# nanoporetech/tombo

Measured on NVIDIA H100. Metric: resquiggle_reads_per_sec, higher is better.
Workload: dtype f64

## Files before the change

### tombo_b200/csrc/batch.h

```cpp
#pragma once
#ifdef TB2_EMUL
#include <stddef.h>
#include "../../include/tombo_b200.h"
struct tb2_ctx;
#else
#include "ctx.h"
#endif

struct ReadState {
    int status;
    int active;
    int done;
    int n_iters;
    int calls;
    int attempt;
    int first_status;
    int use_sv;
    int num_events;
    int n_cpts;
    int rsrtr;
    int n_norm;
    int changed;
    int path;
    int mapped_start, clip;
    int n_stalls;
    int pad_;
    double shc, scc;
    double score;
    tb2_scale_values sv;
};

struct BatchView {
    int n_reads;
    int kmer_width;
    int max_raw;
    const long long *raw_off, *seq_off, *base_off, *ev_off;
    const int *order;
    const unsigned char *seq;
    double *rawf;
    double *norm;
    double *cs;
    double *scores;
    unsigned char *cstate;
    int *cpts;
    double *em;
    double *rm, *rs;
    double *bm;
    double *tmp_b;
    int *starts;
    int *read_tb;
    int *segs_dp;
    int *segs;
    int *stall_ints;
    int stall_cap;
    ReadState *st;
};

struct StagePolicy {
    double outlier_thresh;
    long long max_raw_cpts;
    double min_event_to_seq_ratio;
    double sig_match_thresh;
    int max_scaling_iters;
    int is_rna;
    int skip_seq_scaling;
    double const_scale;
    unsigned int subsample_seed;
    int literal_key;
    int read_index_base;
};

int tb2_launch_prep(tb2_ctx *ctx, const BatchView &b, const void *raw_dev, int raw_dtype,
                    int is_rna, long long total_samples, long long total_bases);
int tb2_launch_begin_call(tb2_ctx *ctx, const BatchView &b, const tb2_params &p,
                          const StagePolicy &pol);
int tb2_launch_normalize(tb2_ctx *ctx, const BatchView &b, const StagePolicy &pol, int first_call);
int tb2_launch_cpts(tb2_ctx *ctx, const BatchView &b, const tb2_params &p, int on_raw);
int tb2_launch_rna_scale(tb2_ctx *ctx, const BatchView &b, const StagePolicy &pol);
int tb2_launch_event_means(tb2_ctx *ctx, const BatchView &b);
int tb2_launch_stalls(tb2_ctx *ctx, const BatchView &b);
int tb2_launch_resolve(tb2_ctx *ctx, const BatchView &b, const tb2_params &p,
                       const StagePolicy &pol, size_t rawdp_cap_doubles);
int tb2_launch_base_means(tb2_ctx *ctx, const BatchView &b);
int tb2_launch_theil_sen(tb2_ctx *ctx, const BatchView &b, const StagePolicy &pol, int first_call);
int tb2_launch_finalize(tb2_ctx *ctx, const BatchView &b, const StagePolicy &pol, int first_call,
                        double *norm_mean_out, double *norm_signal_out);
int tb2_launch_count_active(tb2_ctx *ctx, const BatchView &b, int *dev_counter);

struct BatchResultView {
    int n_reads;
    long long total_bases;
    const double *norm_mean;
    const long long *base_off, *seq_off;
    const unsigned char *seq;
    const int *status;
    int stride;
};
int tb2_batch_result_view(tb2_ctx *ctx, BatchResultView *out);
int tb2_region_accumulate_dev(tb2_ctx *ctx, long long n, const double *stats_dev,
                              const long long *pos_dev, double thresh, double lower, int stat_type);
```

### tombo_b200/csrc/pipeline.cu

```cuda
#include "batch.h"
#include <chrono>
#include <exception>
#include <string>
#include <cstdio>
#include <cstdlib>
#include "kernels.h"
#include <algorithm>
#include <cmath>
#include <cstring>
#include <memory>
#include <vector>

int tb2_launch_start_attempt(tb2_ctx *ctx, const BatchView &b, int attempt);
int tb2_launch_end_call(tb2_ctx *ctx, const BatchView &b, int max_iters);

namespace {

enum {
    B_RAWOFF = 12, B_SEQOFF, B_BASEOFF, B_EVOFF, B_SEQ, B_RAWIN, B_RAWF, B_NORM, B_CS, B_SCORES,
    B_CSTATE, B_CPTS, B_EM, B_RM, B_RS, B_BM, B_TMPB, B_STARTS, B_READTB, B_SEGSDP, B_SEGS,
    B_STALLS, B_STATE, B_DBG, B_COUNTERS, B_OUT_SEGS, B_OUT_NORMMEAN, B_OUT_NORMSIG, B_OUT_SMALL,
    B_SVIN, B_NSTALL, B_ORDER
};

// ... 178 lines not shown
        sv[r] = s.sv;
        score[r] = ok ? s.score : NAN;
        status[r] = s.status;
        n_iters[r] = s.n_iters;
        flags[r] = (s.changed ? 1 : 0) | (s.attempt ? 2 : 0) | ((dbg && dbg[3 * r] == 0) ? 4 : 0);
    }
}

StagePolicy stage_policy(const tb2_policy &pl)
{
    StagePolicy sp;
    sp.outlier_thresh = pl.outlier_thresh;
    sp.max_raw_cpts = pl.max_raw_cpts;
    sp.min_event_to_seq_ratio = pl.min_event_to_seq_ratio;
    sp.sig_match_thresh = pl.sig_match_thresh;
    sp.max_scaling_iters = (int)pl.max_scaling_iters;
    sp.is_rna = (int)pl.is_rna;
    sp.skip_seq_scaling = (int)pl.skip_seq_scaling;
    sp.const_scale = pl.const_scale;
    sp.subsample_seed = pl.subsample_seed;
    sp.literal_key = 0;
    sp.read_index_base = 0;
    return sp;
}

AlignBatch make_align_batch(tb2_ctx *ctx, const BatchView &v, const tb2_params &p, double thresh)
{
    AlignBatch ab;
    ab.n_reads = v.n_reads;
    ab.order = v.order;
    ab.cpts = v.cpts; ab.em = v.em; ab.ev_off = v.ev_off;
    ab.rm = v.rm; ab.rs = v.rs; ab.base_off = v.base_off;
    ab.starts = v.starts; ab.read_tb = v.read_tb; ab.segs = v.segs_dp;
    ab.stride = (int)(sizeof(ReadState) / sizeof(int));
    ab.n_cpts = &v.st[0].n_cpts;
    ab.num_events = &v.st[0].num_events;
    ab.rsrtr = &v.st[0].rsrtr;
    ab.status = &v.st[0].status;
    ab.active = &v.st[0].active;
    ab.dbg = ctx->pool[B_DBG].as<int>();
    ab.params = p;
    ab.sig_match_thresh = thresh;
    return ab;
}

int run_call(tb2_ctx *ctx, const BatchView &v, const tb2_params &p, const StagePolicy &sp,
             const AlignLaunchCfg *acfg ,
             int first_call, double *norm_mean_dev,
             double *norm_sig_dev, size_t rawdp_cap)
{
    int rc;
    if ((rc = tb2_launch_begin_call(ctx, v, p, sp))) return rc;
    if (p.use_t_test_seg) {
        if ((rc = tb2_launch_cpts(ctx, v, p, 1))) return rc;
        if ((rc = tb2_launch_rna_scale(ctx, v, sp))) return rc;
        if ((rc = tb2_launch_normalize(ctx, v, sp, first_call))) return rc;
    } else {
        if ((rc = tb2_launch_normalize(ctx, v, sp, first_call))) return rc;
        if ((rc = tb2_launch_cpts(ctx, v, p, 0))) return rc;
    }
    if ((rc = tb2_launch_event_means(ctx, v))) return rc;
    TB2_CUDA_TRY(ctx, cudaEventRecord(ctx->ev2, ctx->stream));
    for (int k = 0; k < 2; ++k)
        if (acfg[k].tb_words > 0 &&
            (rc = tb2_launch_align(ctx, make_align_batch(ctx, v, p, sp.sig_match_thresh), acfg[k])))
            return rc;
    TB2_CUDA_TRY(ctx, cudaEventRecord(ctx->ev3, ctx->stream));
    if ((rc = tb2_launch_resolve(ctx, v, p, sp, rawdp_cap))) return rc;
    if ((rc = tb2_launch_base_means(ctx, v))) return rc;
    if ((rc = tb2_launch_theil_sen(ctx, v, sp, first_call))) return rc;
    if ((rc = tb2_launch_finalize(ctx, v, sp, first_call, norm_mean_dev, norm_sig_dev))) return rc;
    if ((rc = tb2_launch_end_call(ctx, v, sp.max_scaling_iters))) return rc;
    return TB2_OK;
}

}

extern "C" int tb2_set_model(tb2_ctx *ctx, const double *means, const double *sds, int kmer_width,
                             int central_pos)
{
    int rc = tb2_use(ctx);
    if (rc) return rc;
    if (!means || !sds || kmer_width < 1 || kmer_width > 12 || central_pos < 0 ||
        central_pos >= kmer_width)
        return TB2_ERR_INVALID_ARG;
    const size_t n = (size_t)1 << (2 * kmer_width);
    TB2_CUDA_TRY(ctx, ctx->model_means.reserve(n * 8));
    TB2_CUDA_TRY(ctx, ctx->model_sds.reserve(n * 8));
    TB2_CUDA_TRY(ctx, cudaMemcpyAsync(ctx->model_means.p, means, n * 8, cudaMemcpyHostToDevice, ctx->stream));
    TB2_CUDA_TRY(ctx, cudaMemcpyAsync(ctx->model_sds.p, sds, n * 8, cudaMemcpyHostToDevice, ctx->stream));
    TB2_CUDA_TRY(ctx, cudaStreamSynchronize(ctx->stream));
    ctx->kmer_width = kmer_width;
    ctx->central_pos = central_pos;
    return TB2_OK;
}

namespace {
struct BatchHolder {
    HostBatch hb;
    BatchView v;
    std::vector<int64_t> raw_off;
    int raw_dtype = 0;
    bool uploaded = false, computed = false, has_norm_sig = false;
    bool has_sv_in = false, has_stalls_in = false;
};

BatchHolder *holder_of(tb2_ctx *ctx)
{
    if (!ctx->batch) ctx->batch = std::shared_ptr<void>(new BatchHolder(), [](void *p) { delete (BatchHolder *)p; });
    return (BatchHolder *)ctx->batch.get();
}
}

static int batch_upload_impl(tb2_ctx *ctx, int64_t n_reads, const void *raw, int raw_dtype,
// ... 426 lines not shown
    if (i < n) out[i] = in[i];
}

}

extern "C" int tb2_normalize_raw_signal(tb2_ctx *ctx, const double *raw, int64_t n, int norm_type,
                                        double outlier_thresh, double const_scale,
                                        const tb2_scale_values *sv_in, double *norm_out,
                                        tb2_scale_values *sv_out)
{
    int rc = tb2_use(ctx);
    if (rc) return rc;
    if (!raw || !norm_out || !sv_out || n < 1 || (norm_type != 0 && norm_type != 1))
        return TB2_ERR_INVALID_ARG;
    OneRead o;
    if ((rc = one_read_view(ctx, o, raw, n, 1, default_params(), 2))) return rc;
    ReadState st;
    memset(&st, 0, sizeof(st));
    st.active = 1;
    if (sv_in) { st.use_sv = 1; st.sv = *sv_in; }
    TB2_CUDA_TRY(ctx, cudaMemcpyAsync(o.v.st, &st, sizeof(st), cudaMemcpyHostToDevice, ctx->stream));
    StagePolicy sp;
    memset(&sp, 0, sizeof(sp));
    sp.outlier_thresh = outlier_thresh;
    sp.const_scale = norm_type == 1 ? const_scale : NAN;
    if ((rc = tb2_launch_normalize(ctx, o.v, sp, 1))) return rc;
    TB2_CUDA_TRY(ctx, cudaMemcpyAsync(norm_out, o.v.norm, (size_t)n * 8, cudaMemcpyDeviceToHost, ctx->stream));
    if ((rc = fetch_state(ctx, o.v, &st))) return rc;
    *sv_out = st.sv;
    if (sv_in == nullptr) sv_out->outlier_thresh = outlier_thresh;
    return st.status;
}

extern "C" int tb2_valid_cpts_w_cap(tb2_ctx *ctx, const double *sig, int64_t n,
                                    int64_t min_base_obs, int64_t running_stat_width,
                                    int64_t num_cpts, int t_test, int64_t *cpts_out,
                                    int *read_status)
{
    int rc = tb2_use(ctx);
    if (rc) return rc;
    if (!sig || !cpts_out || n < 1 || num_cpts < 1 || min_base_obs < 1 || running_stat_width < 1)
        return TB2_ERR_INVALID_ARG;
    tb2_params p = default_params();
    p.min_obs_per_base = min_base_obs;
    p.running_stat_width = running_stat_width;
    p.use_t_test_seg = t_test ? 1 : 0;
    OneRead o;
    if ((rc = one_read_view(ctx, o, sig, n, 1, p, num_cpts))) return rc;
    ReadState st;
    memset(&st, 0, sizeof(st));
    st.active = 1;
    st.num_events = (int)num_cpts;
    TB2_CUDA_TRY(ctx, cudaMemcpyAsync(o.v.st, &st, sizeof(st), cudaMemcpyHostToDevice, ctx->stream));
    if ((rc = tb2_launch_cpts(ctx, o.v, p, 1))) return rc;
    if ((rc = fetch_state(ctx, o.v, &st))) return rc;
    if (read_status) *read_status = st.status;
    if (st.status == TB2_OK) {
        std::vector<int> c32((size_t)num_cpts);
        TB2_CUDA_TRY(ctx, cudaMemcpy(c32.data(), o.v.cpts, (size_t)num_cpts * 4, cudaMemcpyDeviceToHost));
        for (int64_t i = 0; i < num_cpts; ++i) cpts_out[i] = c32[i];
    }
    return TB2_OK;
}

extern "C" int tb2_new_means(tb2_ctx *ctx, const double *sig, int64_t n_sig, const int64_t *segs,
                             int64_t n_segs, double *means_out)
{
    int rc = tb2_use(ctx);
    if (rc) return rc;
    if (!sig || !segs || !means_out || n_sig < 1 || n_segs < 1) return TB2_ERR_INVALID_ARG;
    OneRead o;
    if ((rc = one_read_view(ctx, o, nullptr, n_sig, 1, default_params(), n_segs + 1))) return rc;
    TB2_CUDA_TRY(ctx, cudaMemcpyAsync(o.v.norm, sig, (size_t)n_sig * 8, cudaMemcpyHostToDevice, ctx->stream));
    std::vector<int> s32((size_t)n_segs + 1);
    for (int64_t i = 0; i <= n_segs; ++i) {
        if (segs[i] < 0 || segs[i] > n_sig) return TB2_ERR_INVALID_ARG;
        s32[i] = (int)segs[i];
    }
    TB2_CUDA_TRY(ctx, cudaMemcpyAsync(o.v.cpts, s32.data(), (size_t)(n_segs + 1) * 4, cudaMemcpyHostToDevice, ctx->stream));
    ReadState st;
    memset(&st, 0, sizeof(st));
    st.active = 1;
    st.n_cpts = (int)n_segs + 1;
    TB2_CUDA_TRY(ctx, cudaMemcpyAsync(o.v.st, &st, sizeof(st), cudaMemcpyHostToDevice, ctx->stream));
    if ((rc = tb2_launch_event_means(ctx, o.v))) return rc;
    TB2_CUDA_TRY(ctx, cudaMemcpyAsync(means_out, o.v.em, (size_t)n_segs * 8, cudaMemcpyDeviceToHost, ctx->stream));
    TB2_CUDA_TRY(ctx, cudaStreamSynchronize(ctx->stream));
    return TB2_OK;
}

extern "C" int tb2_theil_sen(tb2_ctx *ctx, double prev_shift, double prev_scale,
                             const double *event_means, const double *model_means, int64_t n,
                             uint32_t subsample_key, double *out4, int *read_status)
{
    int rc = tb2_use(ctx);
    if (rc) return rc;
    if (!event_means || !model_means || !out4 || n < 1) return TB2_ERR_INVALID_ARG;
    OneRead o;
    if ((rc = one_read_view(ctx, o, nullptr, 1, n, default_params(), 2))) return rc;
    TB2_CUDA_TRY(ctx, cudaMemcpyAsync(o.v.bm, event_means, (size_t)n * 8, cudaMemcpyHostToDevice, ctx->stream));
    TB2_CUDA_TRY(ctx, cudaMemcpyAsync(o.v.rm, model_means, (size_t)n * 8, cudaMemcpyHostToDevice, ctx->stream));
    ReadState st;
    memset(&st, 0, sizeof(st));
    st.active = 1;
    st.sv.shift = prev_shift; st.sv.scale = prev_scale;
    TB2_CUDA_TRY(ctx, cudaMemcpyAsync(o.v.st, &st, sizeof(st), cudaMemcpyHostToDevice, ctx->stream));
    StagePolicy sp;
// ... 126 lines not shown
```

### tombo_b200/csrc/stage_kernels.cu

```cuda
#include "stage_kernels.cuh"

static inline int grid1d(int n, int bs) { return (n + bs - 1) / bs; }

int tb2_launch_prep(tb2_ctx *ctx, const BatchView &b, const void *raw_dev, int raw_dtype,
                    int is_rna, long long, long long)
{
    if (raw_dtype == 0)
        k_prep<double><<<b.n_reads, ST_THREADS, 0, ctx->stream>>>(
            b, (const double *)raw_dev, is_rna, ctx->model_means.as<double>(),
            ctx->model_sds.as<double>());
    else
        k_prep<short><<<b.n_reads, ST_THREADS, 0, ctx->stream>>>(
            b, (const short *)raw_dev, is_rna, ctx->model_means.as<double>(),
            ctx->model_sds.as<double>());
    TB2_CHECK_LAUNCH(ctx);
    return TB2_OK;
}

int tb2_launch_start_attempt(tb2_ctx *ctx, const BatchView &b, int attempt)
{
    k_start_attempt<<<grid1d(b.n_reads, 256), 256, 0, ctx->stream>>>(b, attempt);
    TB2_CHECK_LAUNCH(ctx);
    return TB2_OK;
}

int tb2_launch_begin_call(tb2_ctx *ctx, const BatchView &b, const tb2_params &p,
                          const StagePolicy &pol)
{
    k_begin_call<<<grid1d(b.n_reads, 256), 256, 0, ctx->stream>>>(b, p, pol);
    TB2_CHECK_LAUNCH(ctx);
    return TB2_OK;
}

int tb2_launch_end_call(tb2_ctx *ctx, const BatchView &b, int max_iters)
{
    k_end_call<<<grid1d(b.n_reads, 256), 256, 0, ctx->stream>>>(b, max_iters);
    TB2_CHECK_LAUNCH(ctx);
    return TB2_OK;
}

int tb2_launch_count_active(tb2_ctx *ctx, const BatchView &b, int *dev_counter)
{
    TB2_CUDA_TRY(ctx, cudaMemsetAsync(dev_counter, 0, 2 * sizeof(int), ctx->stream));
    k_count_active<<<grid1d(b.n_reads, 256), 256, 0, ctx->stream>>>(b, dev_counter);
    TB2_CHECK_LAUNCH(ctx);
    return TB2_OK;
}

int tb2_launch_normalize(tb2_ctx *ctx, const BatchView &b, const StagePolicy &pol, int first_call)
{
    k_normalize<<<b.n_reads, ST_THREADS, 0, ctx->stream>>>(b, pol, first_call);
    TB2_CHECK_LAUNCH(ctx);
    return TB2_OK;
}

int tb2_launch_cpts(tb2_ctx *ctx, const BatchView &b, const tb2_params &p, int on_raw)
{
    if (!p.use_t_test_seg) {
        k_cumsum<<<(b.n_reads + CS_WARPS - 1) / CS_WARPS, CS_WARPS * 32, 0, ctx->stream>>>(b, on_raw);
        TB2_CHECK_LAUNCH(ctx);
    }
    const long long nw = (b.max_raw + 32) / 32;
    long long words = (4 + std::max(0, (int)p.min_obs_per_base - 1)) * nw;
    if (words * 4 > 48 * 1024) words = 0;
    k_cpts<<<b.n_reads, ST_THREADS, (size_t)words * 4, ctx->stream>>>(b, p, on_raw, (int)words);
    TB2_CHECK_LAUNCH(ctx);
    return TB2_OK;
}

int tb2_launch_rna_scale(tb2_ctx *ctx, const BatchView &b, const StagePolicy &pol)
{
    k_rna_scale<<<b.n_reads, ST_THREADS, 0, ctx->stream>>>(b, pol);
    TB2_CHECK_LAUNCH(ctx);
    return TB2_OK;
}

int tb2_launch_event_means(tb2_ctx *ctx, const BatchView &b)
{
    k_event_means<<<b.n_reads, ST_THREADS, 0, ctx->stream>>>(b);
    TB2_CHECK_LAUNCH(ctx);
    return TB2_OK;
}

int tb2_launch_stalls(tb2_ctx *ctx, const BatchView &b)
{
    k_stalls<<<b.n_reads, ST_THREADS, 0, ctx->stream>>>(b);
    TB2_CHECK_LAUNCH(ctx);
    return TB2_OK;
}

int tb2_launch_resolve(tb2_ctx *ctx, const BatchView &b, const tb2_params &p,
                       const StagePolicy &pol, size_t cap)
{
    enum { SLOT_RAWDP = 73, SLOT_CNT2 = 74, SLOT_RAWBIG = 75 };
    const int warps_per_block = 4;
    int grid = ctx->sm_count * 8;
    const int max_useful = (b.n_reads + warps_per_block - 1) / warps_per_block;
    if (grid > max_useful) grid = max_useful > 0 ? max_useful : 1;
    const size_t slots = (size_t)grid * warps_per_block;
    TB2_CUDA_TRY(ctx, ctx->pool[SLOT_RAWDP].reserve(slots * cap * sizeof(double)));
    TB2_CUDA_TRY(ctx, ctx->pool[SLOT_CNT2].reserve(16));
    TB2_CUDA_TRY(ctx, cudaMemsetAsync(ctx->pool[SLOT_CNT2].p, 0, 16, ctx->stream));
    const unsigned long long big_cap = std::min<unsigned long long>(
        (2ULL << 30) / 8, std::max<unsigned long long>((64ULL << 20) / 8, 24ULL * 64ULL * (unsigned long long)std::max(1, b.max_raw)));
    TB2_CUDA_TRY(ctx, ctx->pool[SLOT_RAWBIG].reserve((size_t)big_cap * sizeof(double)));
    k_resolve<<<grid, warps_per_block * 32, 0, ctx->stream>>>(
        b, p, pol, ctx->pool[SLOT_RAWDP].as<double>(), cap, ctx->pool[SLOT_CNT2].as<int>(),
        ctx->pool[SLOT_RAWBIG].as<double>(), big_cap,
        (unsigned long long *)(ctx->pool[SLOT_CNT2].as<int>() + 2));
    TB2_CHECK_LAUNCH(ctx);
    return TB2_OK;
}

int tb2_launch_base_means(tb2_ctx *ctx, const BatchView &b)
{
    k_base_means<<<b.n_reads, ST_THREADS, 0, ctx->stream>>>(b);
    TB2_CHECK_LAUNCH(ctx);
    return TB2_OK;
// ... 35 lines not shown
```

### tombo_b200/csrc/stage_kernels.cuh

```cuda
#pragma once
#include "batch.h"
#include "select.cuh"

#define ST_THREADS TB2_SEL_THREADS

__device__ __forceinline__ bool rd_active(const ReadState &s) { return s.active && s.status == TB2_OK; }

template <class T>
__global__ void __launch_bounds__(ST_THREADS)
k_prep(BatchView b, const T *raw, int is_rna, const double *kmeans, const double *ksds)
{
    const int r = blockIdx.x;
    const long long ro = b.raw_off[r];
    const int n = (int)(b.raw_off[r + 1] - ro);
    for (int i = threadIdx.x; i < n; i += ST_THREADS)
        b.rawf[ro + i] = (double)raw[ro + (is_rna ? n - 1 - i : i)];
    const long long so = b.seq_off[r], bo = b.base_off[r];
    const int nb = (int)(b.base_off[r + 1] - bo);
    const int K = b.kmer_width;
    int bad = 0;
    for (int i = threadIdx.x; i < nb; i += ST_THREADS) {
        int code = 0;
        for (int j = 0; j < K; ++j) {
            const int c = b.seq[so + i + j];
// ... 32 lines not shown
        s.active = 1;
    }
    s.attempt = attempt;
    s.n_iters = 0;
    s.use_sv = 0;
}

__global__ void k_begin_call(BatchView b, tb2_params p, StagePolicy pol)
{
    const int r = blockIdx.x * blockDim.x + threadIdx.x;
    if (r >= b.n_reads) return;
    ReadState &s = b.st[r];
    if (!rd_active(s)) return;
    const int n = (int)(b.raw_off[r + 1] - b.raw_off[r]);
    const int nb = (int)(b.base_off[r + 1] - b.base_off[r]);
    const long long a = (long long)n / p.mean_obs_per_event;
    const long long c = (long long)((double)nb * pol.min_event_to_seq_ratio);
    const long long ne = a > c ? a : c;
    if ((double)ne / (double)p.bandwidth > (double)nb) { s.status = TB2_ERR_TOO_MUCH_SIGNAL; return; }
    if (ne > b.ev_off[r + 1] - b.ev_off[r] || ne < 2) { s.status = TB2_ERR_CAPACITY; return; }
    s.num_events = (int)ne;
}

__global__ void k_end_call(BatchView b, int max_iters)
{
    const int r = blockIdx.x * blockDim.x + threadIdx.x;
    if (r >= b.n_reads) return;
    ReadState &s = b.st[r];
    if (!s.active) return;
    s.calls += 1;
    if (s.status != TB2_OK) { s.active = 0; return; }
    s.n_iters += 1;
    if (s.changed && s.n_iters < max_iters) { s.use_sv = 1; return; }
    s.active = 0;
    s.done = 1;
}

__global__ void k_count_active(BatchView b, int *counters)
{
    const int r = blockIdx.x * blockDim.x + threadIdx.x;
    int act = 0, fail = 0;
    if (r < b.n_reads) {
        act = b.st[r].active != 0;
        fail = (!b.st[r].done && b.st[r].status != TB2_OK);
    }
    act = __syncthreads_count(act);
    fail = __syncthreads_count(fail);
    if (threadIdx.x == 0) {
        if (act) atomicAdd(&counters[0], act);
        if (fail) atomicAdd(&counters[1], fail);
    }
}

__global__ void __launch_bounds__(ST_THREADS)
k_normalize(BatchView b, StagePolicy pol, int first_call)
{
    __shared__ SelectSmem sm;
    const int r = b.order ? b.order[blockIdx.x] : blockIdx.x;
    ReadState &s = b.st[r];
    if (!rd_active(s)) return;
    const long long ro = b.raw_off[r];
    const int n = (int)(b.raw_off[r + 1] - ro);
    const double *raw = b.rawf + ro;
    double *norm = b.norm + ro;
    double shift, scale, lo = NAN, hi = NAN;
    const bool given = s.use_sv != 0;
    const bool use_const = first_call && !isnan(pol.const_scale);
    double mid_a = 0.0, mid_b = 0.0;
    if (!given) {
        auto f_raw = [&](int i) { return raw[i]; };
        if (n & 1) {
            tb2_block_select2(f_raw, PredAll(), n, n / 2, false, &mid_a, &mid_b, sm);
            shift = mid_a;
        } else {
            tb2_block_select2(f_raw, PredAll(), n, n / 2 - 1, true, &mid_a, &mid_b, sm);
            shift = (mid_a + mid_b) / 2.0;
        }
        if (use_const) scale = pol.const_scale;
        else scale = tb2_block_median([&](int i) { return fabs(raw[i] - shift); }, n, sm);
    } else {
        shift = s.sv.shift; scale = s.sv.scale;
    }
    if (scale == 0.0 || isnan(scale)) {
        if (threadIdx.x == 0) s.status = TB2_ERR_UNEXPECTED;
        return;
    }
    for (int i = threadIdx.x; i < n; i += ST_THREADS) norm[i] = (raw[i] - shift) / scale;
    __syncthreads();
    const double thresh = given ? NAN : pol.outlier_thresh;
    if (!isnan(thresh)) {
        double med, mad;
        if ((n & 1) && !use_const) {
            med = 0.0;
            mad = 1.0;
        } else {
            if (n & 1) med = tb2_block_median([&](int i) { return norm[i]; }, n, sm);
            else med = (((mid_a - shift) / scale) + ((mid_b - shift) / scale)) / 2.0;
            mad = tb2_block_median([&](int i) { return fabs(norm[i] - med); }, n, sm);
        }
        lo = med - (mad * thresh);
        hi = med + (mad * thresh);
    } else if (given) { lo = s.sv.lower_lim; hi = s.sv.upper_lim; }
    if (!isnan(lo) && !isnan(hi)) {
        for (int i = threadIdx.x; i < n; i += ST_THREADS) {
            const double v = norm[i];
            norm[i] = v > hi ? hi : (v < lo ? lo : v);
        }
    }
    __syncthreads();
    if (threadIdx.x == 0) {
        s.sv.shift = shift; s.sv.scale = scale; s.sv.lower_lim = lo; s.sv.upper_lim = hi;
        s.sv.outlier_thresh = thresh;
    }
}

__device__ __forceinline__ bool cand_gt(double si, int i, double sk, int k)
{
    return si > sk || (si == sk && i > k);
}

#define CS_WARPS 4
__global__ void __launch_bounds__(CS_WARPS * 32, 8)
k_cumsum(BatchView b, int on_raw)
{
    __shared__ double s_all[CS_WARPS][256];
    const int lane = threadIdx.x & 31, warp = threadIdx.x >> 5;
    const int r = blockIdx.x * CS_WARPS + warp;
    if (r >= b.n_reads) return;
    if (!rd_active(b.st[r])) return;
    double *s_x = s_all[warp];
    const long long ro = b.raw_off[r];
    const int n = (int)(b.raw_off[r + 1] - ro);
    const double *sig = (on_raw ? b.rawf : b.norm) + ro;
    double *cs = b.cs + ro + r;
    double acc = 0.0;
    if (lane == 0) cs[0] = 0.0;
    for (int base = 0; base < n; base += 256) {
#pragma unroll
        for (int q = 0; q < 8; ++q) {
            const int i = base + q * 32 + lane;
            s_x[q * 32 + lane] = (i < n) ? sig[i] : 0.0;
        }
        __syncwarp();
        double mine[8];
#pragma unroll
        for (int q = 0; q < 8; ++q) {
            double m_q = 0.0;
#pragma unroll
            for (int k = 0; k < 32; ++k) {
                acc = acc + s_x[q * 32 + k];
                if (lane == k) m_q = acc;
            }
            mine[q] = m_q;
        }
        __syncwarp();
#pragma unroll
        for (int q = 0; q < 8; ++q) {
            const int i = base + q * 32 + lane;
            if (i < n) cs[i + 1] = mine[q];
        }
    }
}

__device__ __forceinline__ uint32_t cp_shr(const uint32_t *x, int w, int nw, int o)
{
    const uint32_t hi = (w + 1 < nw) ? x[w + 1] : 0u;
    return (x[w] >> o) | (hi << (32 - o));
}
__device__ __forceinline__ uint32_t cp_shl(const uint32_t *x, int w, int o)
{
    const uint32_t lo = (w > 0) ? x[w - 1] : 0u;
    return (x[w] << o) | (lo >> (32 - o));
}

#define CP_MAX_OFF 12

__global__ void __launch_bounds__(ST_THREADS, 5)
k_cpts(BatchView b, tb2_params p, int on_raw, int smem_words)
{
    TB2_DYN_SMEM(uint32_t, cp_smem);
    __shared__ SelectSmem sm;
    __shared__ int s_pos;
    const int r = b.order ? b.order[blockIdx.x] : blockIdx.x;
    ReadState &s = b.st[r];
    if (!rd_active(s)) return;
    const int tid = threadIdx.x, lane = tid & 31, warp = tid >> 5;
    const long long ro = b.raw_off[r];
    const int n = (int)(b.raw_off[r + 1] - ro);
    const double *sig = (on_raw ? b.rawf : b.norm) + ro;
    double *cs = b.cs + ro + r;
    double *sc = b.scores + ro;
    const int w = (int)p.running_stat_width, m = (int)p.min_obs_per_base;
    const int N = s.num_events;
    int n_cand, bound;
    if (!p.use_t_test_seg) {
        n_cand = n + 1 - 2 * w;
        bound = n_cand - 2 * w;
        if (n_cand <= 0) { if (tid == 0) s.status = TB2_ERR_UNEXPECTED; return; }
        for (int i = tid; i < n_cand; i += ST_THREADS)
            sc[i] = fabs(((2 * cs[i + w]) - cs[i]) - cs[i + 2 * w]);
    } else {
        n_cand = n - 2 * w;
        bound = n_cand;
        if (n_cand <= 0) { if (tid == 0) s.status = TB2_ERR_UNEXPECTED; return; }
        for (int pos = tid; pos < n_cand; pos += ST_THREADS) {
            double m1 = 0, m2 = 0, var1 = 0, var2 = 0, d;
            for (int k = 0; k < w; ++k) m1 += sig[pos + k];
            m1 /= (double)w;
            for (int k = 0; k < w; ++k) m2 += sig[pos + w + k];
            m2 /= (double)w;
            for (int k = 0; k < w; ++k) { d = sig[pos + k] - m1; var1 += d * d; }
            for (int k = 0; k < w; ++k) { d = sig[pos + w + k] - m2; var2 += d * d; }
            double t;
            if (var1 + var2 == 0) t = 0.0;
            else if (m1 > m2) t = (m1 - m2) / sqrt(var1 + var2);
            else t = (m2 - m1) / sqrt(var1 + var2);
            sc[pos] = t;
        }
    }
    if (N < 1 || N > n_cand) { if (tid == 0) s.status = (N < 1) ? TB2_ERR_UNEXPECTED : TB2_ERR_FEWER_CPTS; return; }
    __syncthreads();
    const int nw = (n_cand + 31) >> 5;
    const int no = m - 1;
    uint32_t *bits;
    if ((4 + max(no, 0)) * nw <= smem_words) bits = cp_smem;
    else bits = reinterpret_cast<uint32_t *>(b.cstate + ((2 * ro + 128LL * r + 3) & ~3LL));
    if (no > CP_MAX_OFF) { if (tid == 0) s.status = TB2_ERR_CAPACITY; return; }
    uint32_t *A0 = bits, *A1 = bits + nw, *D0 = bits + 2 * nw, *D1 = bits + 3 * nw, *G = bits + 4 * nw;
    for (int wd = warp; wd < nw; wd += ST_THREADS / 32) {
        const int i = wd * 32 + lane;
        const bool valid = i < n_cand;
        const double si = valid ? sc[i] : 0.0;
        for (int o = 1; o <= no; ++o) {
            const bool gt = valid && (i + o < n_cand) && cand_gt(sc[i + o], i + o, si, i);
            const uint32_t g = __ballot_sync(TB2_FULL_MASK, gt);
            if (lane == 0) G[(o - 1) * nw + wd] = g;
        }
        const uint32_t inv = __ballot_sync(TB2_FULL_MASK, !valid);
        if (lane == 0) { A0[wd] = 0u; D0[wd] = inv; }
    }
    __syncthreads();
    uint32_t *Ac = A0, *An = A1, *Dc = D0, *Dn = D1;
    for (;;) {
        int undecided = 0;
        for (int wd = tid; wd < nw; wd += ST_THREADS) {
            const uint32_t a = Ac[wd], dd = Dc[wd];
            const uint32_t U = ~dd;
            uint32_t na = a, nd = dd;
            if (U != 0u) {
                uint32_t accnb = 0u, blocked = 0u;
                for (int o = 1; o <= no; ++o) {
                    const uint32_t *Go = G + (o - 1) * nw;
                    accnb |= cp_shr(Ac, wd, nw, o) | cp_shl(Ac, wd, o);
                    const uint32_t d_hi = (wd + 1 < nw) ? Dc[wd + 1] : ~0u;
                    const uint32_t d_lo = (wd > 0) ? Dc[wd - 1] : ~0u;
                    const uint32_t u_up = ~((dd >> o) | (d_hi << (32 - o)));
                    const uint32_t u_dn = ~((dd << o) | (d_lo >> (32 - o)));
// ... 48 lines not shown
    } else {
        auto f_pos = [&](int i) { return (double)i; };
        auto p_tie = [&](int i) { return p_acc(i) && sc[i] == vN; };
        double pv, pd;
        tb2_block_select2(f_pos, p_tie, n_cand, (int)e - need, false, &pv, &pd, sm);
        posN = (int)pv;
    }
    if (eq_all > 1u) {
        unsigned int h2 = 0;
        for (int i = tid; i < n_cand; i += ST_THREADS) h2 += (sc[i] == vN && i > posN);
        higher += tb2_block_sum(h2, sm);
    }
    if (N > 1 && (int)higher + 1 >= bound) { if (tid == 0) s.status = TB2_ERR_FEWER_CPTS; return; }
    const int *si = b.stall_ints ? b.stall_ints + 2 * (size_t)b.stall_cap * r : nullptr;
    const int ns = b.stall_ints ? s.n_stalls : 0;
    for (int wd = warp; wd < nw; wd += ST_THREADS / 32) {
        const int i = wd * 32 + lane;
        bool keep = (A[wd] >> lane) & 1u;
        if (keep) {
            const double v = sc[i];
            keep = v > vN || (v == vN && i >= posN);
            const int c = i + w;
            for (int k = 0; keep && k < ns; ++k) if (si[2 * k] < c && c < si[2 * k + 1]) keep = false;
        }
        const uint32_t kw = __ballot_sync(TB2_FULL_MASK, keep);
        if (lane == 0) K[wd] = kw;
    }
    __syncthreads();
    const int per = (nw + ST_THREADS - 1) / ST_THREADS;
    const int w0 = min(nw, tid * per), w1 = min(nw, w0 + per);
    unsigned int mine = 0;
    for (int wd = w0; wd < w1; ++wd) mine += __popc(K[wd]);
    unsigned int inc = mine;
#pragma unroll
    for (int off = 1; off < 32; off <<= 1) {
        const unsigned int o = __shfl_up_sync(TB2_FULL_MASK, inc, off);
        if (lane >= off) inc += o;
    }
    if (lane == 31) sm.warp_tot[warp] = inc;
    __syncthreads();
    unsigned int base = 0, total = 0;
    for (int q = 0; q < ST_THREADS / 32; ++q) { if (q < warp) base += sm.warp_tot[q]; total += sm.warp_tot[q]; }
    unsigned int o = base + inc - mine;
    int *cp = b.cpts + b.ev_off[r];
    for (int wd = w0; wd < w1; ++wd) {
        uint32_t kw = K[wd];
        while (kw) {
            const int bit = __ffs(kw) - 1;
            kw &= kw - 1u;
            cp[o++] = wd * 32 + bit + w;
        }
    }
    if (tid == 0) s.n_cpts = (int)total;
}

__global__ void __launch_bounds__(ST_THREADS) k_event_means(BatchView b)
{
    const int r = blockIdx.x;
    const ReadState &s = b.st[r];
    if (!rd_active(s)) return;
    const double *norm = b.norm + b.raw_off[r];
    const int *cp = b.cpts + b.ev_off[r];
    double *em = b.em + b.ev_off[r];
    const int ne = s.n_cpts - 1;
    if (ne < 1) { if (threadIdx.x == 0) b.st[r].status = TB2_ERR_UNEXPECTED; return; }
    for (int e = threadIdx.x; e < ne; e += ST_THREADS) {
        const int a = cp[e], z = cp[e + 1];
        double acc = 0;
        for (int k = a; k < z; ++k) acc += norm[k];
        em[e] = acc / (double)(z - a);
    }
}

__global__ void __launch_bounds__(ST_THREADS) k_rna_scale(BatchView b, StagePolicy pol)
{
    __shared__ SelectSmem sm;
    const int r = blockIdx.x;
    ReadState &s = b.st[r];
    if (!rd_active(s) || s.use_sv == 1) return;
    if (!isnan(pol.const_scale)) return;
    const double *raw = b.rawf + b.raw_off[r];
    const int *cp = b.cpts + b.ev_off[r];
    double *em = b.em + b.ev_off[r];
    int ne = 10000;
    if ((double)s.n_cpts * 0.75 < (double)ne) ne = (int)((double)s.n_cpts * 0.75);
    if (ne < 2) { if (threadIdx.x == 0) s.status = TB2_ERR_UNEXPECTED; return; }
    for (int e = threadIdx.x; e < ne - 1; e += ST_THREADS) {
        const int a = cp[e], z = cp[e + 1];
        double acc = 0;
        for (int k = a; k < z; ++k) acc += raw[k];
        em[e] = acc / (double)(z - a);
    }
    __syncthreads();
    const double med = tb2_block_median([&](int i) { return em[i]; }, ne - 1, sm);
    const double mad = tb2_block_median([&](int i) { return fabs(em[i] - med); }, ne - 1, sm);
    __syncthreads();
    if (threadIdx.x == 0) {
        s.sv.shift = med; s.sv.scale = mad;
        s.sv.lower_lim = -pol.outlier_thresh; s.sv.upper_lim = pol.outlier_thresh;
        s.sv.outlier_thresh = NAN;
        s.use_sv = 2;
    }
}

__global__ void __launch_bounds__(ST_THREADS) k_stalls(BatchView b)
{
    const int r = blockIdx.x;
    ReadState &s = b.st[r];
    if (s.done) return;
    const int tid = threadIdx.x;
    const long long ro = b.raw_off[r];
    const int n = (int)(b.raw_off[r + 1] - ro);
    const double *raw = b.rawf + ro;
    double *cs = b.cs + ro + r;
    double *metric = b.scores + ro;
    volatile unsigned char *below = b.cstate + ro;
    const int window = 350, mini = 50, nwin = 7, min_consec = 200, edge = 100;
    const double thresh = 40;
    if (tid == 0) s.n_stalls = 0;
    if (n < window) return;
    if (tid < 32) {
        double acc = 0.0;
        for (int base = 0; base < n; base += 32) {
            const double x = (base + tid < n) ? raw[base + tid] : 0.0;
// ... 976 lines not shown
```

Measured before the change: 685,000.

## Fuse normalization, cumsum and change-point scores into streamed warp kernel

For the non-t-test path, normalization, cumulative sum and windowed score computation are fused into one warp-per-read kernel that keeps a ring-buffered cumsum in shared memory, so the full cs array is never written to global memory. Scale-value derivation becomes its own kernel on the first call. The change-point kernel now caches scores in shared memory for short reads and computes event means inline, which removes the separate event-means launch. In exchange, the fused kernel runs one warp per read, which may cut parallelism for long reads, and the larger shared-memory use can lower occupancy.

```diff
diff --git a/tombo_b200/csrc/batch.h b/tombo_b200/csrc/batch.h
--- a/tombo_b200/csrc/batch.h
+++ b/tombo_b200/csrc/batch.h
@@ -75,7 +75,9 @@
 int tb2_launch_begin_call(tb2_ctx *ctx, const BatchView &b, const tb2_params &p,
                           const StagePolicy &pol);
 int tb2_launch_normalize(tb2_ctx *ctx, const BatchView &b, const StagePolicy &pol, int first_call);
-int tb2_launch_cpts(tb2_ctx *ctx, const BatchView &b, const tb2_params &p, int on_raw);
+int tb2_launch_norm_scores(tb2_ctx *ctx, const BatchView &b, const StagePolicy &pol, int first_call,
+                           int w);
+int tb2_launch_cpts(tb2_ctx *ctx, const BatchView &b, const tb2_params &p, int on_raw, int streamed);
 int tb2_launch_rna_scale(tb2_ctx *ctx, const BatchView &b, const StagePolicy &pol);
 int tb2_launch_event_means(tb2_ctx *ctx, const BatchView &b);
 int tb2_launch_stalls(tb2_ctx *ctx, const BatchView &b);
diff --git a/tombo_b200/csrc/pipeline.cu b/tombo_b200/csrc/pipeline.cu
--- a/tombo_b200/csrc/pipeline.cu
+++ b/tombo_b200/csrc/pipeline.cu
@@ -254,14 +254,14 @@
     int rc;
     if ((rc = tb2_launch_begin_call(ctx, v, p, sp))) return rc;
     if (p.use_t_test_seg) {
-        if ((rc = tb2_launch_cpts(ctx, v, p, 1))) return rc;
+        if ((rc = tb2_launch_cpts(ctx, v, p, 1, 0))) return rc;
         if ((rc = tb2_launch_rna_scale(ctx, v, sp))) return rc;
         if ((rc = tb2_launch_normalize(ctx, v, sp, first_call))) return rc;
+        if ((rc = tb2_launch_event_means(ctx, v))) return rc;
     } else {
-        if ((rc = tb2_launch_normalize(ctx, v, sp, first_call))) return rc;
-        if ((rc = tb2_launch_cpts(ctx, v, p, 0))) return rc;
-    }
-    if ((rc = tb2_launch_event_means(ctx, v))) return rc;
+        if ((rc = tb2_launch_norm_scores(ctx, v, sp, first_call, (int)p.running_stat_width))) return rc;
+        if ((rc = tb2_launch_cpts(ctx, v, p, 0, 1))) return rc;
+    }
     TB2_CUDA_TRY(ctx, cudaEventRecord(ctx->ev2, ctx->stream));
     for (int k = 0; k < 2; ++k)
         if (acfg[k].tb_words > 0 &&
@@ -794,7 +794,7 @@
     st.active = 1;
     st.num_events = (int)num_cpts;
     TB2_CUDA_TRY(ctx, cudaMemcpyAsync(o.v.st, &st, sizeof(st), cudaMemcpyHostToDevice, ctx->stream));
-    if ((rc = tb2_launch_cpts(ctx, o.v, p, 1))) return rc;
+    if ((rc = tb2_launch_cpts(ctx, o.v, p, 1, 0))) return rc;
     if ((rc = fetch_state(ctx, o.v, &st))) return rc;
     if (read_status) *read_status = st.status;
     if (st.status == TB2_OK) {
diff --git a/tombo_b200/csrc/stage_kernels.cu b/tombo_b200/csrc/stage_kernels.cu
--- a/tombo_b200/csrc/stage_kernels.cu
+++ b/tombo_b200/csrc/stage_kernels.cu
@@ -54,16 +54,41 @@
     return TB2_OK;
 }
 
-int tb2_launch_cpts(tb2_ctx *ctx, const BatchView &b, const tb2_params &p, int on_raw)
+int tb2_launch_norm_scores(tb2_ctx *ctx, const BatchView &b, const StagePolicy &pol, int first_call,
+                           int w)
 {
-    if (!p.use_t_test_seg) {
+    if (first_call) {
+        k_scale_values<<<b.n_reads, ST_THREADS, 0, ctx->stream>>>(b, pol);
+        TB2_CHECK_LAUNCH(ctx);
+    }
+    if (w < 1) { ctx->err = "running_stat_width must be positive"; return TB2_ERR_INVALID_ARG; }
+    int ring = 512;
+    while (ring < 256 + 2 * w) ring <<= 1;
+    const size_t smem = (size_t)NS_WARPS * ring * sizeof(double);
+    if (smem > 160 * 1024) { ctx->err = "running_stat_width too large"; return TB2_ERR_CAPACITY; }
+    TB2_CUDA_TRY(ctx, cudaFuncSetAttribute(k_norm_scores, cudaFuncAttributeMaxDynamicSharedMemorySize,
+                                           (int)smem));
+    k_norm_scores<<<(b.n_reads + NS_WARPS - 1) / NS_WARPS, NS_WARPS * 32, smem, ctx->stream>>>(b, w, ring);
+    TB2_CHECK_LAUNCH(ctx);
+    return TB2_OK;
+}
+
+#define CP_SMEM_SCORES 4200
+
+int tb2_launch_cpts(tb2_ctx *ctx, const BatchView &b, const tb2_params &p, int on_raw, int streamed)
+{
+    if (!p.use_t_test_seg && !streamed) {
         k_cumsum<<<(b.n_reads + CS_WARPS - 1) / CS_WARPS, CS_WARPS * 32, 0, ctx->stream>>>(b, on_raw);
         TB2_CHECK_LAUNCH(ctx);
     }
     const long long nw = (b.max_raw + 32) / 32;
     long long words = (4 + std::max(0, (int)p.min_obs_per_base - 1)) * nw;
     if (words * 4 > 48 * 1024) words = 0;
-    k_cpts<<<b.n_reads, ST_THREADS, (size_t)words * 4, ctx->stream>>>(b, p, on_raw, (int)words);
+    const int sc_cap = p.use_t_test_seg ? 0 : std::min(b.max_raw + 1, CP_SMEM_SCORES);
+    const size_t smem = (size_t)((words + 1) & ~1LL) * 4 + (size_t)sc_cap * sizeof(double);
+    TB2_CUDA_TRY(ctx, cudaFuncSetAttribute(k_cpts, cudaFuncAttributeMaxDynamicSharedMemorySize,
+                                           (int)smem));
+    k_cpts<<<b.n_reads, ST_THREADS, smem, ctx->stream>>>(b, p, on_raw, (int)words, sc_cap, streamed);
     TB2_CHECK_LAUNCH(ctx);
     return TB2_OK;
 }
diff --git a/tombo_b200/csrc/stage_kernels.cuh b/tombo_b200/csrc/stage_kernels.cuh
--- a/tombo_b200/csrc/stage_kernels.cuh
+++ b/tombo_b200/csrc/stage_kernels.cuh
@@ -108,6 +108,48 @@
     }
 }
 
+__device__ bool tb2_derive_scale_values(const double *raw, int n, const StagePolicy &pol,
+                                        bool use_const, SelectSmem &sm, tb2_scale_values *v)
+{
+    double shift, scale, lo = NAN, hi = NAN;
+    double mid_a = 0.0, mid_b = 0.0;
+    auto f_raw = [&](int i) { return raw[i]; };
+    if (n & 1) {
+        tb2_block_select2(f_raw, PredAll(), n, n / 2, false, &mid_a, &mid_b, sm);
+        shift = mid_a;
+    } else {
+        tb2_block_select2(f_raw, PredAll(), n, n / 2 - 1, true, &mid_a, &mid_b, sm);
+        shift = (mid_a + mid_b) / 2.0;
+    }
+    if (use_const) scale = pol.const_scale;
+    else scale = tb2_block_median([&](int i) { return fabs(raw[i] - shift); }, n, sm);
+    if (scale == 0.0 || isnan(scale)) return false;
+    const double thresh = pol.outlier_thresh;
+    if (!isnan(thresh)) {
+        double med, mad;
+        if ((n & 1) && !use_const) {
+            med = 0.0;
+            mad = 1.0;
+        } else {
+            auto f_norm = [&](int i) { return (raw[i] - shift) / scale; };
+            if (n & 1) med = tb2_block_median(f_norm, n, sm);
+            else med = (((mid_a - shift) / scale) + ((mid_b - shift) / scale)) / 2.0;
+            mad = tb2_block_median([&](int i) { return fabs(f_norm(i) - med); }, n, sm);
+        }
+        lo = med - (mad * thresh);
+        hi = med + (mad * thresh);
+    }
+    v->shift = shift; v->scale = scale; v->lower_lim = lo; v->upper_lim = hi;
+    v->outlier_thresh = thresh;
+    return true;
+}
+
+__device__ __forceinline__ double tb2_norm_of(double x, const tb2_scale_values &v, bool clip)
+{
+    const double y = (x - v.shift) / v.scale;
+    return clip ? (y > v.upper_lim ? v.upper_lim : (y < v.lower_lim ? v.lower_lim : y)) : y;
+}
+
 __global__ void __launch_bounds__(ST_THREADS)
 k_normalize(BatchView b, StagePolicy pol, int first_call)
 {
@@ -119,60 +161,60 @@
     const int n = (int)(b.raw_off[r + 1] - ro);
     const double *raw = b.rawf + ro;
     double *norm = b.norm + ro;
-    double shift, scale, lo = NAN, hi = NAN;
-    const bool given = s.use_sv != 0;
-    const bool use_const = first_call && !isnan(pol.const_scale);
-    double mid_a = 0.0, mid_b = 0.0;
-    if (!given) {
-        auto f_raw = [&](int i) { return raw[i]; };
-        if (n & 1) {
-            tb2_block_select2(f_raw, PredAll(), n, n / 2, false, &mid_a, &mid_b, sm);
-            shift = mid_a;
-        } else {
-            tb2_block_select2(f_raw, PredAll(), n, n / 2 - 1, true, &mid_a, &mid_b, sm);
-            shift = (mid_a + mid_b) / 2.0;
-        }
-        if (use_const) scale = pol.const_scale;
-        else scale = tb2_block_median([&](int i) { return fabs(raw[i] - shift); }, n, sm);
+    tb2_scale_values v = s.sv;
+    if (s.use_sv == 0) {
+        if (!tb2_derive_scale_values(raw, n, pol, first_call && !isnan(pol.const_scale), sm, &v)) {
+            if (threadIdx.x == 0) s.status = TB2_ERR_UNEXPECTED;
+            return;
+        }
     } else {
-        shift = s.sv.shift; scale = s.sv.scale;
-    }
-    if (scale == 0.0 || isnan(scale)) {
-        if (threadIdx.x == 0) s.status = TB2_ERR_UNEXPECTED;
-        return;
-    }
-    for (int i = threadIdx.x; i < n; i += ST_THREADS) norm[i] = (raw[i] - shift) / scale;
+        v.outlier_thresh = NAN;
+        if (v.scale == 0.0 || isnan(v.scale)) {
+            if (threadIdx.x == 0) s.status = TB2_ERR_UNEXPECTED;
+            return;
+        }
+    }
+    const bool clip = !isnan(v.lower_lim) && !isnan(v.upper_lim);
+    for (int i = threadIdx.x; i < n; i += ST_THREADS) norm[i] = tb2_norm_of(raw[i], v, clip);
     __syncthreads();
-    const double thresh = given ? NAN : pol.outlier_thresh;
-    if (!isnan(thresh)) {
-        double med, mad;
-        if ((n & 1) && !use_const) {
-            med = 0.0;
-            mad = 1.0;
-        } else {
-            if (n & 1) med = tb2_block_median([&](int i) { return norm[i]; }, n, sm);
-            else med = (((mid_a - shift) / scale) + ((mid_b - shift) / scale)) / 2.0;
-            mad = tb2_block_median([&](int i) { return fabs(norm[i] - med); }, n, sm);
-        }
-        lo = med - (mad * thresh);
-        hi = med + (mad * thresh);
-    } else if (given) { lo = s.sv.lower_lim; hi = s.sv.upper_lim; }
-    if (!isnan(lo) && !isnan(hi)) {
-        for (int i = threadIdx.x; i < n; i += ST_THREADS) {
-            const double v = norm[i];
-            norm[i] = v > hi ? hi : (v < lo ? lo : v);
-        }
-    }
-    __syncthreads();
+    if (threadIdx.x == 0) s.sv = v;
+}
+
+__global__ void __launch_bounds__(ST_THREADS)
+k_scale_values(BatchView b, StagePolicy pol)
+{
+    __shared__ SelectSmem sm;
+    const int r = b.order ? b.order[blockIdx.x] : blockIdx.x;
+    ReadState &s = b.st[r];
+    if (!rd_active(s) || s.use_sv != 0) return;
+    const long long ro = b.raw_off[r];
+    tb2_scale_values v;
+    const bool ok = tb2_derive_scale_values(b.rawf + ro, (int)(b.raw_off[r + 1] - ro), pol,
+                                            !isnan(pol.const_scale), sm, &v);
     if (threadIdx.x == 0) {
-        s.sv.shift = shift; s.sv.scale = scale; s.sv.lower_lim = lo; s.sv.upper_lim = hi;
-        s.sv.outlier_thresh = thresh;
+        if (ok) s.sv = v;
+        else s.status = TB2_ERR_UNEXPECTED;
     }
 }
 
 __device__ __forceinline__ bool cand_gt(double si, int i, double sk, int k)
 {
     return si > sk || (si == sk && i > k);
+}
+
+__device__ __forceinline__ void tb2_warp_cumsum_tile(const double *t, int lane, double &acc,
+                                                     double mine[8])
+{
+#pragma unroll
+    for (int q = 0; q < 8; ++q) {
+        double m_q = 0.0;
+#pragma unroll
+        for (int k = 0; k < 32; ++k) {
+            acc = acc + t[q * 32 + k];
+            if (lane == k) m_q = acc;
+        }
+        mine[q] = m_q;
+    }
 }
 
 #define CS_WARPS 4
@@ -199,16 +241,7 @@
         }
         __syncwarp();
         double mine[8];
-#pragma unroll
-        for (int q = 0; q < 8; ++q) {
-            double m_q = 0.0;
-#pragma unroll
-            for (int k = 0; k < 32; ++k) {
-                acc = acc + s_x[q * 32 + k];
-                if (lane == k) m_q = acc;
-            }
-            mine[q] = m_q;
-        }
+        tb2_warp_cumsum_tile(s_x, lane, acc, mine);
         __syncwarp();
 #pragma unroll
         for (int q = 0; q < 8; ++q) {
@@ -218,6 +251,74 @@
     }
 }
 
+#define NS_WARPS 4
+__global__ void __launch_bounds__(NS_WARPS * 32, 8)
+k_norm_scores(BatchView b, int w, int ring)
+{
+    TB2_DYN_SMEM(double, ns_smem);
+    const int lane = threadIdx.x & 31, warp = threadIdx.x >> 5;
+    const int r = blockIdx.x * NS_WARPS + warp;
+    if (r >= b.n_reads) return;
+    ReadState &s = b.st[r];
+    if (!rd_active(s)) return;
+    const tb2_scale_values v = s.sv;
+    if (s.use_sv != 0) {
+        if (v.scale == 0.0 || isnan(v.scale)) {
+            __syncwarp();
+            if (lane == 0) s.status = TB2_ERR_UNEXPECTED;
+            return;
+        }
+        if (lane == 0) s.sv.outlier_thresh = NAN;
+    }
+    const bool clip = !isnan(v.lower_lim) && !isnan(v.upper_lim);
+    const long long ro = b.raw_off[r];
+    const int n = (int)(b.raw_off[r + 1] - ro);
+    const double *raw = b.rawf + ro;
+    double *norm = b.norm + ro;
+    double *cs = ns_smem + (size_t)warp * ring;
+    const int M = ring - 1;
+    double *sc = b.scores + ro;
+    double acc = 0.0;
+    if (lane == 0) cs[M] = 0.0;
+    int i_done = 0;
+    for (int base = 0; base < n; base += 256) {
+        double *t = cs + (base & M);
+#pragma unroll
+        for (int q = 0; q < 8; ++q) {
+            const int i = base + q * 32 + lane;
+            double x = 0.0;
+            if (i < n) {
+                x = tb2_norm_of(raw[i], v, clip);
+                norm[i] = x;
+            }
+            t[q * 32 + lane] = x;
+        }
+        __syncwarp();
+        double mine[8];
+        tb2_warp_cumsum_tile(t, lane, acc, mine);
+        __syncwarp();
+#pragma unroll
+        for (int q = 0; q < 8; ++q) t[q * 32 + lane] = mine[q];
+        __syncwarp();
+        const int i_hi = min(n, base + 256) - 2 * w + 1;
+        for (int i = i_done + lane; i < i_hi; i += 32)
+            sc[i] = fabs(((2 * cs[(i + w - 1) & M]) - cs[(i - 1) & M]) - cs[(i + 2 * w - 1) & M]);
+        i_done = max(i_done, i_hi);
+        __syncwarp();
+    }
+}
+
+__device__ __forceinline__ void tb2_event_means(const double *norm, const int *cp, double *em,
+                                                int ne, int t0, int stride)
+{
+    for (int e = t0; e < ne; e += stride) {
+        const int a = cp[e], z = cp[e + 1];
+        double acc = 0;
+        for (int k = a; k < z; ++k) acc += norm[k];
+        em[e] = acc / (double)(z - a);
+    }
+}
+
 __device__ __forceinline__ uint32_t cp_shr(const uint32_t *x, int w, int nw, int o)
 {
     const uint32_t hi = (w + 1 < nw) ? x[w + 1] : 0u;
@@ -232,7 +333,7 @@
 #define CP_MAX_OFF 12
 
 __global__ void __launch_bounds__(ST_THREADS, 5)
-k_cpts(BatchView b, tb2_params p, int on_raw, int smem_words)
+k_cpts(BatchView b, tb2_params p, int on_raw, int smem_words, int sc_cap = 0, int streamed = 0)
 {
     TB2_DYN_SMEM(uint32_t, cp_smem);
     __shared__ SelectSmem sm;
@@ -243,22 +344,28 @@
     const int tid = threadIdx.x, lane = tid & 31, warp = tid >> 5;
     const long long ro = b.raw_off[r];
     const int n = (int)(b.raw_off[r + 1] - ro);
-    const double *sig = (on_raw ? b.rawf : b.norm) + ro;
-    double *cs = b.cs + ro + r;
-    double *sc = b.scores + ro;
     const int w = (int)p.running_stat_width, m = (int)p.min_obs_per_base;
     const int N = s.num_events;
-    int n_cand, bound;
+    const int n_cand = p.use_t_test_seg ? n - 2 * w : n + 1 - 2 * w;
+    if (n_cand <= 0) { if (tid == 0) s.status = TB2_ERR_UNEXPECTED; return; }
+    double *sc = b.scores + ro;
+    if (n_cand <= sc_cap) {
+        double *s_sc = reinterpret_cast<double *>(cp_smem + ((smem_words + 1) & ~1));
+        if (streamed)
+            for (int i = tid; i < n_cand; i += ST_THREADS) s_sc[i] = sc[i];
+        sc = s_sc;
+    }
+    int bound;
     if (!p.use_t_test_seg) {
-        n_cand = n + 1 - 2 * w;
         bound = n_cand - 2 * w;
-        if (n_cand <= 0) { if (tid == 0) s.status = TB2_ERR_UNEXPECTED; return; }
-        for (int i = tid; i < n_cand; i += ST_THREADS)
-            sc[i] = fabs(((2 * cs[i + w]) - cs[i]) - cs[i + 2 * w]);
+        if (!streamed) {
+            const double *cs = b.cs + ro + r;
+            for (int i = tid; i < n_cand; i += ST_THREADS)
+                sc[i] = fabs(((2 * cs[i + w]) - cs[i]) - cs[i + 2 * w]);
+        }
     } else {
-        n_cand = n - 2 * w;
+        const double *sig = (on_raw ? b.rawf : b.norm) + ro;
         bound = n_cand;
-        if (n_cand <= 0) { if (tid == 0) s.status = TB2_ERR_UNEXPECTED; return; }
         for (int pos = tid; pos < n_cand; pos += ST_THREADS) {
             double m1 = 0, m2 = 0, var1 = 0, var2 = 0, d;
             for (int k = 0; k < w; ++k) m1 += sig[pos + k];
@@ -413,6 +520,11 @@
         }
     }
     if (tid == 0) s.n_cpts = (int)total;
+    if (!streamed) return;
+    const int ne = (int)total - 1;
+    if (ne < 1) { if (tid == 0) s.status = TB2_ERR_UNEXPECTED; return; }
+    __syncthreads();
+    tb2_event_means(b.norm + ro, cp, b.em + b.ev_off[r], ne, tid, ST_THREADS);
 }
 
 __global__ void __launch_bounds__(ST_THREADS) k_event_means(BatchView b)
@@ -420,17 +532,10 @@
     const int r = blockIdx.x;
     const ReadState &s = b.st[r];
     if (!rd_active(s)) return;
-    const double *norm = b.norm + b.raw_off[r];
-    const int *cp = b.cpts + b.ev_off[r];
-    double *em = b.em + b.ev_off[r];
     const int ne = s.n_cpts - 1;
     if (ne < 1) { if (threadIdx.x == 0) b.st[r].status = TB2_ERR_UNEXPECTED; return; }
-    for (int e = threadIdx.x; e < ne; e += ST_THREADS) {
-        const int a = cp[e], z = cp[e + 1];
-        double acc = 0;
-        for (int k = a; k < z; ++k) acc += norm[k];
-        em[e] = acc / (double)(z - a);
-    }
+    tb2_event_means(b.norm + b.raw_off[r], b.cpts + b.ev_off[r], b.em + b.ev_off[r], ne,
+                    threadIdx.x, ST_THREADS);
 }
 
 __global__ void __launch_bounds__(ST_THREADS) k_rna_scale(BatchView b, StagePolicy pol)
```

Measured after the change: 694,600 (median of 6 runs). 1.01x the previous value.
